# huyhoang17/DB_text_minimal

Hardware: AMD Instinct MI355X
Metric: train images/sec @640x640 bs=16/GPU (higher is better)
Workload: dtype f32

## Files before the change

db_text_minimal_amd/_lib.py:

```python
import ctypes
import os
import subprocess

_HERE = os.path.dirname(os.path.abspath(__file__))
LIB_PATH = os.environ.get('DBN_LIB_PATH') or os.path.join(_HERE, 'libdbnet_hip.so')
CSRC = os.path.join(_HERE, 'csrc')

_P, _I, _L, _F = ctypes.c_void_p, ctypes.c_int, ctypes.c_long, ctypes.c_float

SIGNATURES = {
    'dbn_pack_weights': 'piiiiiipp',
    'dbn_igemm_panel_floats': 'iiiiii',
    'dbn_igemm_packed_floats': 'ii',
    'dbn_igemm_f32': 'pppp' + 'i' * 14 + 'p',
    'dbn_igemm_tile_config': 'ii',
    'dbn_igemm_tile_config_ns': 'iii',
    'dbn_conv_bn_ws_floats': 'iiiiii',
    'dbn_pack_weights_batched': 'piip',
    'dbn_igemm_splitk_plan': 'iiii',
    'dbn_igemm_splitk_plan_ns': 'iiiii',
    'dbn_igemm_splitk_f32': 'pppp' + 'i' * 16 + 'pp',
    'dbn_deform_im2col': 'ppp' + 'i' * 11 + 'p',
    'dbn_deform_col2im': 'ppppp' + 'i' + 'p' + 'i' * 11 + 'p',
    'dbn_deform_col2im_ws_bytes': 'i' * 8,
# ... 180 lines not shown
    'dbn_convt16_rows': '',
    'dbn_convt16_panel_bytes': '',
    'dbn_convt16_eligible': 'iiiiii',
    'dbn_convt16_pack': 'ippp',
    'dbn_convt16_bn_t': 'ippppiii' + 'pp' + 'ff' + 'ppppppp' + 'p',
    'dbn_stem16_padded_h': 'i',
    'dbn_stem16_padded_w': 'i',
    'dbn_stem16_rows': '',
    'dbn_stem16_panel_bytes': '',
    'dbn_stem16_eligible': 'iiii',
    'dbn_stem16_pack': 'ippp',
    'dbn_nchw3_to_padded4_t': 'ipppiiip',
    'dbn_stem16_conv_bn_t': 'ipppiii' + 'pp' + 'ff' + 'ppppppp' + 'p',
    'dbn_head_tail_fwd_t': 'i' + SIGNATURES['dbn_head_tail_fwd'],
    'dbn_head_tail_bwd_t': 'i' + SIGNATURES['dbn_head_tail_bwd'],
})
LONG_RETURN = {'dbn_jpeg_coef_elems', 'dbn_jpeg_dhuff_ws_bytes', 'dbn_jpeg_encode_bound', 'dbn_greedy_decode_ws_bytes', 'dbn_det_eval_ws_bytes', 'dbn_detect_ws_bytes', 'dbn_detect_poly_ws_bytes', 'dbn_detect_poly_verts_cap', 'dbn_mfma_sustained_flops', 'dbn_conv_bn_final_group_doubles', 'dbn_maxpool_bn_backward_ws_floats', 'dbn_pw16_panel_bytes', 'dbn_stem16_panel_bytes', 'dbn_convt16_panel_bytes', 'dbn_winograd_panel_floats', 'dbn_winograd_wgrad_slab_floats', 'dbn_winograd_ws_floats', 'dbn_igemm_splitk_slab_floats', 'dbn_deform_col2im_ws_bytes', 'dbn_deform_col2im_gather_ws_bytes', 'dbn_igemm_bn_final_counters', 'dbn_igemm_bn_final_group_floats', 'dbn_igemm_panel_floats_t', 'dbn_wgrad_slab_floats_hw', 'dbn_wgrad_slab_floats', 'dbn_igemm_panel_floats', 'dbn_igemm_bf16s_panel_floats', 'dbn_db_loss_ohem_ws_bytes', 'dbn_conv_bn_ws_floats', 'dbn_pyramid_conv_ws_floats'}
_KIND = {'p': _P, 'i': _I, 'l': _L, 'f': _F}


class HipLibraryError(RuntimeError):
    pass


class WgradReduceJob(ctypes.Structure):
    _fields_ = ([('slab', _P), ('grad', _P)] + [(f, _I) for f in ('splitk', 'O', 'J', 'Jp', 'BM', 'BN', 'Cb', 'I', 'RS', 'G', 'natural', 'blocks')]
                + [('scale', _F), ('smem_bytes', _I)])


class BnbFinal(ctypes.Structure):
# ... 52 lines not shown
```

db_text_minimal_amd/csrc/common.h:

```cpp
#pragma once
#include <hip/hip_runtime.h>
#include <stdint.h>

typedef float f32x4 __attribute__((ext_vector_type(4)));
typedef float f32x16 __attribute__((ext_vector_type(16)));

#include <stdlib.h>

#ifdef DBN_EXPERIMENTS
#define DBN_HAS_EXPERIMENTS 1
static inline int dbn_env_int(const char* name, int dflt) { const char* e = getenv(name); return e ? atoi(e) : dflt; }
static inline double dbn_env_double(const char* name, double dflt) { const char* e = getenv(name); return e ? atof(e) : dflt; }
#else
#define DBN_HAS_EXPERIMENTS 0
static inline constexpr int dbn_env_int(const char*, int dflt) { return dflt; }
static inline constexpr double dbn_env_double(const char*, double dflt) { return dflt; }
#endif

#ifndef DBN_RACE
#define DBN_RACE 0
#endif
#if DBN_RACE
__device__ __forceinline__ void dbn_race_jitter(unsigned site) {
    unsigned h = (threadIdx.x >> 6) * 2654435761u + blockIdx.x * 40503u + site * 2246822519u;
// ... 60 lines not shown
    const float* row = part + idx * nb;
    double s = 0.0;
    int b = lane32;
    for (; b + 96 < nb; b += 128) {
        const float v0 = row[b], v1 = row[b + 32], v2 = row[b + 64], v3 = row[b + 96];
        s += ((double)v0 + (double)v1) + ((double)v2 + (double)v3);
    }
    for (; b < nb; b += 32) s += (double)row[b];
#pragma unroll
    for (int o = 16; o > 0; o >>= 1) s += __shfl_xor(s, o, 64);
    return s;
}

__device__ __forceinline__ float dbn_affine(float y, float sc, float sh) { return fmaf(y, sc, sh); }
__device__ __forceinline__ float dbn_affine_relu(float y, float sc, float sh) { return fmaxf(fmaf(y, sc, sh), 0.f); }

#define DBN_AT_F32 0
#define DBN_AT_BF16 1
#define DBN_AT_F16 2
typedef unsigned dbn_u32x2 __attribute__((ext_vector_type(2)));
typedef _Float16 dbn_f16x4 __attribute__((ext_vector_type(4)));
typedef __bf16 dbn_bf16x2 __attribute__((ext_vector_type(2)));

__host__ __device__ constexpr int dbn_esize(int at) { return at == 0 ? 4 : 2; }

template <int AT>
__device__ __forceinline__ f32x4 dbn_ld4(const void* __restrict__ p, long i4) {
    if constexpr (AT == 0) {
        return reinterpret_cast<const f32x4*>(p)[i4];
    } else if constexpr (AT == 1) {
// ... 86 lines not shown
```

db_text_minimal_amd/csrc/head_loss.hip:

```cpp
#include "common.h"

namespace {

__device__ __forceinline__ float sigmoidf_(float x) { return 1.f / (1.f + __expf(-x)); }
__device__ __forceinline__ float sigmoid_acc(float x) { return 1.f / (1.f + expf(-x)); }
__device__ __forceinline__ float sigmoid_fast(float x) { return __builtin_amdgcn_rcpf(1.f + __expf(-x)); }

template <int CTRL>
__device__ __forceinline__ float dpp_f32(float v) {
    return __builtin_bit_cast(float, __builtin_amdgcn_update_dpp(0, __builtin_bit_cast(int, v), CTRL, 0xF, 0xF, true));
}
constexpr int DPP_QUAD_XOR1 = 0xB1;
constexpr int DPP_QUAD_XOR2 = 0x4E;
constexpr int DPP_ROW_HALF_MIRROR = 0x141;
constexpr int DPP_ROW_MIRROR = 0x140;
__device__ __forceinline__ float group16_sum(float v) {
    v += dpp_f32<DPP_QUAD_XOR1>(v);
    v += dpp_f32<DPP_QUAD_XOR2>(v);
    v += dpp_f32<DPP_ROW_HALF_MIRROR>(v);
    v += dpp_f32<DPP_ROW_MIRROR>(v);
    return v;
}
#ifndef DBN_HT_NODPP
#define DBN_HT_NODPP 0
// ... 122 lines not shown
        }
    }
    for (; px < r1; px += gstride, advance()) {
        f32x4 vb[NQ], vt[NQ];
        load(xb, px, vb);
        load(xt, px, vt);
        finish(vb, vt, n, hq, wq);
    }
}

#if DBN_HT_WAVES
#define DBN_HT_OCC __attribute__((amdgpu_waves_per_eu(DBN_HT_WAVES, DBN_HT_WAVES)))
#else
#define DBN_HT_OCC
#endif
template <int AT>
__global__ __launch_bounds__(256) DBN_HT_OCC void head_tail_bwd_kernel(const void* __restrict__ xb, const void* __restrict__ xt, const float* __restrict__ wb,
                                     const float* __restrict__ wt, const float* __restrict__ preds,
                                     const float* __restrict__ dpreds, const float* __restrict__ sc_b,
                                     const float* __restrict__ sh_b, const float* __restrict__ sc_t,
                                     const float* __restrict__ sh_t, const float* __restrict__ mean_b,
                                     const float* __restrict__ rstd_b, const float* __restrict__ mean_t,
                                     const float* __restrict__ rstd_t, void* __restrict__ dxb, void* __restrict__ dxt,
                                     float* __restrict__ part, int N, int Hq, int Wq, int CH, float kstep) {
    const int q = threadIdx.x & 15;
    const int grp = threadIdx.x >> 4;
    const bool bn = sc_b != nullptr;
    f32x4 scb = {1.f, 1.f, 1.f, 1.f}, shb = {0.f, 0.f, 0.f, 0.f}, sct = scb, sht = shb;
    if (bn) {
        scb = *reinterpret_cast<const f32x4*>(sc_b + 4 * q);
        shb = *reinterpret_cast<const f32x4*>(sh_b + 4 * q);
        sct = *reinterpret_cast<const f32x4*>(sc_t + 4 * q);
        sht = *reinterpret_cast<const f32x4*>(sh_t + 4 * q);
    }
    const long npx = (long)N * Hq * Wq;
    const long gstride = (long)gridDim.x * (blockDim.x >> 4);
    f32x4 wbq[4], wtq[4];
#pragma unroll
    for (int e = 0; e < 4; ++e) {
// ... 52 lines not shown
        const f32x4 lb = {quad_bcast<0>(dlb), quad_bcast<1>(dlb), quad_bcast<2>(dlb), quad_bcast<3>(dlb)};
        const f32x4 lt = {quad_bcast<0>(dlt), quad_bcast<1>(dlt), quad_bcast<2>(dlt), quad_bcast<3>(dlt)};
        f32x4 vb = dbn_ld4<AT>(xb, px * 16 + q);
        f32x4 vt = dbn_ld4<AT>(xt, px * 16 + q);
        const f32x4 yb = vb, yt = vt;
        if (bn) {
#pragma unroll
            for (int e = 0; e < 4; ++e) {
                vb[e] = dbn_affine_relu(vb[e], scb[e], shb[e]);
                vt[e] = dbn_affine_relu(vt[e], sct[e], sht[e]);
            }
        }
        f32x4 gb, gt;
#pragma unroll
        for (int e = 0; e < 4; ++e) {
            gb[e] = wbq[e][0] * lb[0] + wbq[e][1] * lb[1] + wbq[e][2] * lb[2] + wbq[e][3] * lb[3];
            gt[e] = wtq[e][0] * lt[0] + wtq[e][1] * lt[1] + wtq[e][2] * lt[2] + wtq[e][3] * lt[3];
            awb[e] += vb[e] * lb;
            awt[e] += vt[e] * lt;
        }
        dbn_st4<AT>(dxb, px * 16 + q, gb);
        dbn_st4<AT>(dxt, px * 16 + q, gt);
        if (bnsum) {
            if constexpr (AT != 0) {
#pragma unroll
                for (int e = 0; e < 4; ++e) {
                    gb[e] = AT == 1 ? (float)(__bf16)gb[e] : (float)(_Float16)gb[e];
                    gt[e] = AT == 1 ? (float)(__bf16)gt[e] : (float)(_Float16)gt[e];
                }
            }
#pragma unroll
            for (int e = 0; e < 4; ++e) {
                const float mb = vb[e] > 0.f ? gb[e] : 0.f, mt = vt[e] > 0.f ? gt[e] : 0.f;
                s1b[e] += mb;
                s2b[e] += mb * ((yb[e] - mub[e]) * rsb[e]);
                s1t[e] += mt;
                s2t[e] += mt * ((yt[e] - mut[e]) * rst[e]);
// ... 540 lines not shown
        hipLaunchKernelGGL((head_tail_fwd_kernel<0, 16>), grid, dim3(256), 0, (hipStream_t)stream, xb, xt, wb, wt, bias_b, bias_t, bn_scale_b,
                           bn_shift_b, bn_scale_t, bn_shift_t, out, N, Hq, Wq, channels, kstep, per);
    else
        return DBN_ERR_ARG;
    return dbn_status();
}
int dbn_head_tail_fwd(const float* xb, const float* xt, const float* wb, const float* wt, const float* bias_b,
                      const float* bias_t, const float* bn_scale_b, const float* bn_shift_b, const float* bn_scale_t,
                      const float* bn_shift_t, float* out, int N, int Hq, int Wq, int channels, float kstep, void* stream) {
    return dbn_head_tail_fwd_t(0, xb, xt, wb, wt, bias_b, bias_t, bn_scale_b, bn_shift_b, bn_scale_t, bn_shift_t, out, N, Hq, Wq,
                               channels, kstep, stream);
}

int dbn_head_tail_bwd_ws_floats() { return 2048 * (2 * 257 + 4 * 64); }

int dbn_head_tail_bwd_t(int at, const void* xb, const void* xt, const float* wb, const float* wt, const float* preds,
                        const float* dpreds, const float* bn_scale_b, const float* bn_shift_b, const float* bn_scale_t,
                        const float* bn_shift_t, const float* bn_mean_b, const float* bn_rstd_b, const float* bn_mean_t,
                        const float* bn_rstd_t, float* bn_sums, void* dxb, void* dxt, float* dw_b, float* dbias_b, float* dw_t,
                        float* dbias_t, int N, int Hq, int Wq, int channels, float kstep, float grad_scale, float* ws, void* stream) {
    DBN_REQUIRE(xb && xt && wb && wt && preds && dpreds && dxb && dxt && dw_b && dbias_b && dw_t && dbias_t && ws);
    DBN_REQUIRE((bn_scale_b && bn_shift_b && bn_scale_t && bn_shift_t) || (!bn_scale_b && !bn_shift_b && !bn_scale_t && !bn_shift_t));
    DBN_REQUIRE(channels == 2 || channels == 3);
    const bool sums = bn_sums != nullptr;
    DBN_REQUIRE(!sums || (bn_scale_b && bn_mean_b && bn_rstd_b && bn_mean_t && bn_rstd_t));
    hipStream_t st = (hipStream_t)stream;
    const long npx = (long)N * Hq * Wq;
    const int nb = dbn_grid(npx * 16, 256, 2047);
    DBN_DISPATCH_AT(at, hipLaunchKernelGGL(head_tail_bwd_kernel<AT>, dim3(nb), dim3(256), 0, st, xb, xt, wb, wt, preds, dpreds, bn_scale_b,
                                           bn_shift_b, bn_scale_t, bn_shift_t, sums ? bn_mean_b : nullptr, bn_rstd_b, bn_mean_t,
                                           bn_rstd_t, dxb, dxt, ws, N, Hq, Wq, channels, kstep));
    hipLaunchKernelGGL(fold_head_grads_kernel, dim3(dbn_ceil_div(2 * 257, 8)), dim3(256), 0, st, ws, nb, dw_b, dbias_b, dw_t, dbias_t,
                       grad_scale);
    if (sums)
        hipLaunchKernelGGL(fold_partials_d_kernel, dim3(dbn_ceil_div(256, 8)), dim3(256), 0, st, ws + (long)514 * nb, nb, 256, bn_sums,
                           1.0f);
    return dbn_status();
}

int dbn_head_tail_bwd(const float* xb, const float* xt, const float* wb, const float* wt, const float* preds,
                      const float* dpreds, const float* bn_scale_b, const float* bn_shift_b, const float* bn_scale_t,
                      const float* bn_shift_t, const float* bn_mean_b, const float* bn_rstd_b, const float* bn_mean_t,
                      const float* bn_rstd_t, float* bn_sums, float* dxb, float* dxt, float* dw_b, float* dbias_b, float* dw_t,
                      float* dbias_t, int N, int Hq, int Wq, int channels, float kstep, float grad_scale, float* ws, void* stream) {
    return dbn_head_tail_bwd_t(0, xb, xt, wb, wt, preds, dpreds, bn_scale_b, bn_shift_b, bn_scale_t, bn_shift_t, bn_mean_b, bn_rstd_b,
                               bn_mean_t, bn_rstd_t, bn_sums, dxb, dxt, dw_b, dbias_b, dw_t, dbias_t, N, Hq, Wq, channels, kstep,
                               grad_scale, ws, stream);
}

static const long DB_LOSS_PART_BYTES = 1024L * NSUM * 8;
int dbn_db_loss_ws_bytes() { return (int)DB_LOSS_PART_BYTES + 64; }

// ... 96 lines not shown
```

db_text_minimal_amd/csrc/pointwise.hip:

```cpp
#include "common.h"

namespace {

constexpr int MAX_PART = 1024;
constexpr int STREAM_BLOCKS = 768;
constexpr int UNROLL = 4;

constexpr int CHUNK_C = 1024;

template <int NV, class F>
__device__ __forceinline__ void channel_reduce(int M, int Cfull, float* __restrict__ part, F&& body) {
    const int cb = blockIdx.y * CHUNK_C, C = min(CHUNK_C, Cfull - cb);
    const int c4n = C >> 2, cq = cb >> 2;
    const int c4 = threadIdx.x % c4n, rl = threadIdx.x / c4n;
    const int nrl = blockDim.x / c4n;
    const int rows_per = (M + gridDim.x - 1) / gridDim.x;
    const int r0 = blockIdx.x * rows_per, r1 = min(M, r0 + rows_per);
    f32x4 acc[NV];
#pragma unroll
    for (int v = 0; v < NV; ++v) acc[v] = f32x4{0.f, 0.f, 0.f, 0.f};
    if (rl < nrl) {
#pragma unroll 4
        for (int r = r0 + rl; r < r1; r += nrl) body(r, cq + c4, acc);
    }
// ... 217 lines not shown
    s1 = red[0][0];
    s2 = red[1][0];
    dbeta[c] = (float)(s1 * gscale);
    dgamma[c] = (float)(s2 * gscale);
    c1[c] = (float)(s1 / M);
    c2[c] = (float)(s2 / M);
}

template <int AT>
__device__ __forceinline__ float round_to_storage(float v) {
    if constexpr (AT == 1) return (float)(__bf16)v;
    else if constexpr (AT == 2) return (float)(_Float16)v;
    else return v;
}

template <int AT, int QW>
__global__ __launch_bounds__(256) void bn_bwd_apply_kernel(const void* __restrict__ y, const void* __restrict__ zmask,
                                                           const float* __restrict__ msc, const float* __restrict__ msh,
                                                           const void* __restrict__ dout, const float* __restrict__ mean,
                                                           const float* __restrict__ rstd, const float* __restrict__ gamma,
                                                           const float* __restrict__ c1, const float* __restrict__ c2,
                                                           void* __restrict__ dy, void* __restrict__ gout, int gout_acc,
                                                           long total, int C, float* __restrict__ bias_part) {
    static_assert(QW == 1 || (QW == 2 && AT != 0), "two quads per access: 16-bit storage");
    const int cin = C / (4 * QW);
    const long i0 = blockIdx.x * (long)blockDim.x + threadIdx.x;
    const long stride = (long)gridDim.x * blockDim.x;
    const int c = (int)(i0 % cin) * 4 * QW;
    const f32x4 zero = {0.f, 0.f, 0.f, 0.f};
    f32x4 s_[QW], h_[QW], mu[QW], rs[QW], k1[QW], k2[QW], gr[QW], bsum[QW];
#pragma unroll
    for (int q = 0; q < QW; ++q) {
        s_[q] = h_[q] = zero;
        if (msc) {
            s_[q] = *reinterpret_cast<const f32x4*>(msc + c + 4 * q);
            h_[q] = *reinterpret_cast<const f32x4*>(msh + c + 4 * q);
        }
        mu[q] = *reinterpret_cast<const f32x4*>(mean + c + 4 * q);
        rs[q] = *reinterpret_cast<const f32x4*>(rstd + c + 4 * q);
        k1[q] = *reinterpret_cast<const f32x4*>(c1 + c + 4 * q);
        k2[q] = *reinterpret_cast<const f32x4*>(c2 + c + 4 * q);
        gr[q] = *reinterpret_cast<const f32x4*>(gamma + c + 4 * q) * rs[q];
        bsum[q] = zero;
    }
    const bool acc = gout && gout_acc;
    auto ld = [&](const void* ptr, long i, f32x4 (&v)[QW]) {
        if constexpr (QW == 1) v[0] = dbn_ld4<AT>(ptr, i);
        else dbn_ldq<AT>(ptr, i, v);
    };
    auto st = [&](void* ptr, long i, const f32x4 (&v)[QW]) {
        if constexpr (QW == 1) dbn_st4<AT>(ptr, i, v[0]);
        else dbn_stq<AT>(ptr, i, v);
    };
    auto one = [&](long i, f32x4 (&g)[QW], const f32x4 (&v)[QW], const f32x4 (&z)[QW], const f32x4 (&old)[QW]) {
        f32x4 d[QW], go[QW];
#pragma unroll
        for (int q = 0; q < QW; ++q) {
            if (zmask) {
#pragma unroll
                for (int e = 0; e < 4; ++e) g[q][e] = z[q][e] > 0.f ? g[q][e] : 0.f;
            } else if (msc) {
#pragma unroll
                for (int e = 0; e < 4; ++e) g[q][e] = dbn_affine(v[q][e], s_[q][e], h_[q][e]) > 0.f ? g[q][e] : 0.f;
            }
            const f32x4 xh = (v[q] - mu[q]) * rs[q];
            d[q] = gr[q] * (g[q] - k1[q] - xh * k2[q]);
#pragma unroll
            for (int e = 0; e < 4; ++e) {
                float t = d[q][e];
                asm("" : "+v"(t));
// ... 2 lines not shown
            bsum[q] += d[q];
            go[q] = acc ? g[q] + old[q] : g[q];
        }
        st(dy, i, d);
        if (gout) st(gout, i, go);
    };
    auto zeros = [&](f32x4 (&v)[QW]) {
#pragma unroll
        for (int q = 0; q < QW; ++q) v[q] = zero;
    };
    long i = i0;
    for (; i + (UNROLL - 1) * stride < total; i += UNROLL * stride) {
        f32x4 g[UNROLL][QW], v[UNROLL][QW], z[UNROLL][QW], o[UNROLL][QW];
#pragma unroll
        for (int u = 0; u < UNROLL; ++u) {
            ld(dout, i + u * stride, g[u]);
            ld(y, i + u * stride, v[u]);
        }
#pragma unroll
        for (int u = 0; u < UNROLL; ++u) {
            if (zmask) ld(zmask, i + u * stride, z[u]);
            else zeros(z[u]);
            if (acc) ld(gout, i + u * stride, o[u]);
            else zeros(o[u]);
        }
#pragma unroll
        for (int u = 0; u < UNROLL; ++u) one(i + u * stride, g[u], v[u], z[u], o[u]);
    }
    for (; i < total; i += stride) {
        f32x4 g[QW], v[QW], z[QW], o[QW];
        ld(dout, i, g);
        ld(y, i, v);
        if (zmask) ld(zmask, i, z);
        else zeros(z);
        if (acc) ld(gout, i, o);
        else zeros(o);
        one(i, g, v, z, o);
    }
    if (bias_part) {
        __shared__ f32x4 red[QW][256];
#pragma unroll
        for (int q = 0; q < QW; ++q) red[q][threadIdx.x] = bsum[q];
        __syncthreads();
        if ((int)threadIdx.x < cin) {
            const int cq = (int)((blockIdx.x * (long)blockDim.x + threadIdx.x) % cin) * 4 * QW;
#pragma unroll
// ... 785 lines not shown
        } else if (sums) {
            hipLaunchKernelGGL(bn_bwd_finalize_kernel, dim3(dbn_ceil_div(C, 8)), dim3(256), 0, st, sums, sums_parts > 0 ? sums_parts : 1, M,
                               C, dgamma, dbeta, c1, c2, grad_scale);
        } else {
            hipLaunchKernelGGL(bn_bwd_reduce_kernel<AT>, red_grid(nbu, C), dim3(256), red_smem(C, 2), st, y, zmask, mask_scale,
                               mask_shift, dout, save_mean, save_rstd, M, C, ws);
            hipLaunchKernelGGL(bn_bwd_finalize_kernel, dim3(dbn_ceil_div(C, 8)), dim3(256), 0, st, ws, nbu, M, C, dgamma, dbeta, c1, c2,
                               grad_scale);
        }
#ifndef DBN_DBG_SKIP_BN_BWD_APPLY
#define DBN_DBG_SKIP_BN_BWD_APPLY 0
#endif
        if constexpr (AT != 0) {
            if (wide && !DBN_DBG_SKIP_BN_BWD_APPLY)
                hipLaunchKernelGGL((bn_bwd_apply_kernel<AT, 2>), dim3(grid), dim3(256), 0, st, y, zmask, mask_scale, mask_shift, dout, save_mean,
                                   save_rstd, gamma, c1, c2, dy, gout, gout_accumulate, total4, C, dbias_conv ? ws : nullptr);
        }
        if (!wide && !DBN_DBG_SKIP_BN_BWD_APPLY)
            hipLaunchKernelGGL((bn_bwd_apply_kernel<AT, 1>), dim3(grid), dim3(256), 0, st, y, zmask, mask_scale, mask_shift, dout, save_mean,
                               save_rstd, gamma, c1, c2, dy, gout, gout_accumulate, total4, C, dbias_conv ? ws : nullptr);
    });
    if (dbias_conv)
        hipLaunchKernelGGL(fold_partials_kernel, dim3(dbn_ceil_div(C, 8)), dim3(256), 0, st, ws, grid, C, dbias_conv, grad_scale);
    return dbn_status();
}

int dbn_bn_backward(const float* y, const float* zmask, const float* mask_scale, const float* mask_shift, const float* dout,
                    const float* save_mean, const float* save_rstd, const float* gamma, float* dy, float* gout, int gout_accumulate,
                    float* dgamma, float* dbeta, int M, int C, float grad_scale, float* ws, void* stream) {
    return dbn_bn_backward_t(0, nullptr, 0, y, zmask, mask_scale, mask_shift, dout, save_mean, save_rstd, gamma, dy, gout, gout_accumulate,
                             dgamma, dbeta, nullptr, M, C, grad_scale, ws, stream);
}

int dbn_bn_backward_from_sums(const float* sums, const float* y, const float* zmask, const float* mask_scale, const float* mask_shift,
                              const float* dout, const float* save_mean, const float* save_rstd, const float* gamma, float* dy,
                              float* gout, int gout_accumulate, float* dgamma, float* dbeta, int M, int C, float grad_scale,
// ... 264 lines not shown
```

db_text_minimal_amd/engine.py:

```python
import contextlib
import os

import torch

from . import _lib
from ._lib import check

DEAD_PREFIXES = ('backbone.fc.', 'backbone.smooth.')
K_STEP_DEFAULT = 50.0


def _p(t):
    return None if t is None else t.data_ptr()


def flat_layout(numels):
    offs, total = [], 0
    for n in numels:
        offs.append(total)
        total += (n + 3) // 4 * 4
    return offs, total


IGEMM_TILE_NAMES = {1: 'igemm_f32_kernel<128,128,2,2,%d,%d,%d,%s,%d,%s>', 2: 'igemm_f32_kernel<256,64,4,1,%d,%d,%d,%s,%d,%s>',
# ... 1051 lines not shown
            at, srcp = self._src(x.data_ptr(), C)
            check(self.L.dbn_igemm_act_t(at, self.ns, srcp, wpk.data_ptr(), vconv.bias.data_ptr(), _p(res), int(relu), z.data_ptr(), N, H, W, C,
                                         Ho, Wo, conv.cout, k, k, s, p, 0, 0, self.stream), 'igemm act ' + name)
        if self.prof:
            self.prof.end()
        return z

    apply_on_load = os.environ.get('DBN_APPLY_ON_LOAD', '1') == '1'
    fpn_level0_winograd = os.environ.get('DBN_FPN_LV0_WINOGRAD', '1') == '1'

    def lazy_act(self, y, convs, train):
        return all(self.plan(conv, y.shape, train, fp32_tensors=y.dtype == torch.float32).apply_on_load for conv in convs)

    bias_grad_in_bn = True

    def bn_backward(self, name, y, mask, dout, dy_name, gout=None, gout_acc=False, sums=None, conv_bias=None, sums_parts=1):
        self._flush_wgrads()
        C = y.shape[-1]
        M = y.numel() // C
        dy = self.buf(dy_name, *y.shape)
        zmask = msc = msh = None
        if isinstance(mask, str):
            msc, msh = self.bufs[name + '/scale'], self.bufs[name + '/shift']
        elif mask is not None:
            zmask = mask
        if sums is None and name in self._bnb_sums:
            sums, sums_parts = self._bnb_sums.pop(name)
        dbias = None
        if conv_bias is not None and self.bias_grad_in_bn and 256 % (C // 4) == 0:
            dbias = self.grad_views[conv_bias]
            self._bias_done.add(conv_bias)
        nb = y.numel() * y.element_size()
        rd = 2 + (zmask is not None)
        self._prof_hbm('bn_bwd_reduce_kernel + bn_bwd_finalize_kernel + bn_bwd_apply_kernel', nb * ((0 if sums is not None else rd) + rd + 1 + (gout is not None) * (1 + bool(gout_acc))),
                       name + (' [sums given]' if sums is not None else ''))
        check(self.L.dbn_bn_backward_t(self.at, _p(sums), int(sums_parts), y.data_ptr(), _p(zmask), _p(msc), _p(msh), dout.data_ptr(),
                                        self.bufs[name + '/mean'].data_ptr(), self.bufs[name + '/rstd'].data_ptr(),
                                        self.views[name + '.weight'].data_ptr(), dy.data_ptr(), _p(gout), int(gout_acc),
                                        self.grad_views[name + '.weight'].data_ptr(), self.grad_views[name + '.bias'].data_ptr(),
                                        _p(dbias), M, C, self.grad_scale, self.reduce_ws().data_ptr(), self.stream),
              'bn backward ' + name)
        if self.prof:
            self.prof.end()
        return dy

    def up_fwd(self, src, addend, dst, coff=0):
        N, Hs, Ws, C = src.shape
        _, H, W, Cd = dst.shape
# ... 454 lines not shown
            check(self.L.dbn_winograd_conv_act_f32(zs[0].data_ptr(), up.data_ptr(), vconv.bias.data_ptr(), None, 0, z.data_ptr(), N, H, W, Cg, Co,
                                                   self.stream), 'winograd ' + name)
            if self.prof:
                self.prof.end()
        if self.prof:
            flops = sum(2.0 * N * t.shape[1] * t.shape[2] * Cg * Co * ((1 << g) + 2)**2 for g, t in enumerate(zs) if g >= first)
            bn_tile = 256 if self.L.dbn_pyramid_wide_would_run(self.at, N, H, W, Cg, Co) else 128
            waves = '1,4' if (self.at in (1, 2) and self.ns == 1) else '2,2'
            self.prof.begin('igemm_f32_kernel<128,%d,%s,3,%d,%d,false,0,true>' % (bn_tile, waves, self.ns, self.at), flops, 0.0, 'fwd %s (pyramid)' % name)
        check(self.L.dbn_pyramid_conv_act_t(first, self.at, *[t.data_ptr() for t in zs], *[w_.data_ptr() for w_ in wpk], vconv.bias.data_ptr(), 1,
                                            z.data_ptr(), N, H, W, Cg, Co, self.ns, self.stream), 'pyramid_conv_act')
        if self.prof:
            self.prof.end()
        return z

    def backward(self, dpreds):
        if self.saved_generation != self.generation:
            raise RuntimeError('backward() without a matching train-mode forward (activations were overwritten)')
        m, L, st = self.model, self.L, self.stream
        N, H, W, Hh, Wh, resample = self.saved_shape
        B = self.bufs
        self._bias_done = set()
        self._bnb_sums = {}
        self._dcn_read_back()
        self._wgrad_fifo, self._reduce_pending = [], []
        self._slab_free = [None, None]
        out = self.saved_out
        dpreds = dpreds.contiguous()
        assert dpreds.shape == (N, 3, H, W)
        if resample:
            dhead = self.fbuf('head/dout', *out.shape)
            check(L.dbn_bilinear_bwd(dpreds.data_ptr(), dhead.data_ptr(), N * 3, 2 * Hh, 2 * Wh, H, W, st), 'bilinear_bwd')
            dpreds = dhead
        head = m.segmentation_head
        b6, t6 = head.binarize[6], head.thresh[6]
        dz1b = self.buf('binarize/dz1', N, Hh, Wh, 64)
        dz1t = self.buf('thresh/dz1', N, Hh, Wh, 64)
        ws = self.scratch('_head_ws', L.dbn_head_tail_bwd_ws_floats())
        G = self.grad_views
        hb, ht = 'segmentation_head.binarize.4', 'segmentation_head.thresh.4'
        bn_sums = self.fbuf('head/bn4_sums', 4, 64)
        self._prof_hbm('head_tail_bwd_kernel + fold_head_grads_kernel + fold_partials_d_kernel', 4.0 * dz1b.element_size() * dz1b.numel() + 4.0 * (out.numel() + dpreds.numel()))
        check(L.dbn_head_tail_bwd_t(self.at, B['binarize/y1'].data_ptr(), B['thresh/y1'].data_ptr(), b6.weight.data_ptr(),
                                  t6.weight.data_ptr(), out.data_ptr(), dpreds.data_ptr(), B[hb + '/scale'].data_ptr(),
                                  B[hb + '/shift'].data_ptr(), B[ht + '/scale'].data_ptr(), B[ht + '/shift'].data_ptr(),
                                  B[hb + '/mean'].data_ptr(), B[hb + '/rstd'].data_ptr(), B[ht + '/mean'].data_ptr(),
                                  B[ht + '/rstd'].data_ptr(), bn_sums.data_ptr(), dz1b.data_ptr(), dz1t.data_ptr(),
                                  G['segmentation_head.binarize.6.weight'].data_ptr(),
                                  G['segmentation_head.binarize.6.bias'].data_ptr(),
                                  G['segmentation_head.thresh.6.weight'].data_ptr(),
                                  G['segmentation_head.thresh.6.bias'].data_ptr(), N, Hh, Wh, 3, float(head.k),
                                  self.grad_scale, ws.data_ptr(), st), 'head_tail_bwd')
        if self.prof:
            self.prof.end()
        f, f_act = B.get('fpn/z'), None
        if f is None:
            f, f_act = B['fpn/y'], (B['segmentation_body.conv.1/scale'], B['segmentation_body.conv.1/shift'])
        df = self.buf('fpn/dz', *f.shape)
        fpn = m.segmentation_body
        pre = 'segmentation_body.'
        for i, (br, dz1) in enumerate((('binarize', dz1b), ('thresh', dz1t))):
            seq = getattr(head, br)
            hp = 'segmentation_head.%s.' % br
            dy1 = self.bn_backward(hp + '4', B[br + '/y1'], 'self', dz1, br + '/dy1', sums=bn_sums[2 * i:2 * i + 2],
                                   conv_bias=hp + '3.bias' if seq[3].bias is not None else None)
            dz0 = self.buf(br + '/dz0', *B[br + '/z0'].shape)
            self.convT_bwd(hp + '3', dy1, B[br + '/z0'], seq[3], dz0, consumer=(hp + '1', B[br + '/y0'], None))
            dy0 = self.bn_backward(hp + '1', B[br + '/y0'], 'self', dz0, br + '/dy0',
                                   conv_bias=hp + '0.bias' if seq[0].bias is not None else None)
            self.conv_wgrad(hp + '0', dy0, f, seq[0], x_act=f_act)
            self.conv_dgrad(hp + '0', dy0, seq[0], df, accumulate=(i > 0),
                            consumer=(pre + 'conv.1', B['fpn/y'], None) if i > 0 else None)
        fpn = m.segmentation_body
        pre = 'segmentation_body.'
        dfy = self.bn_backward(pre + 'conv.1', B['fpn/y'], 'self', df, 'fpn/dy',
                               conv_bias=pre + 'conv.0.bias' if fpn.conv[0].bias is not None else None)
        dP = {}
        levels = ('smooth_p2', 'smooth_p3', 'smooth_p4', 'reduce_conv_c5')
        zs = [B[nm + '/z'] for nm in levels]
        if self.fpn_exact:
# ... 277 lines not shown
```

include/dbnet_hip.h:

```cpp
#ifndef DBNET_HIP_H
#define DBNET_HIP_H
#ifdef __cplusplus
extern "C" {
#endif


int dbn_pack_weights(const float* w_oihw, int O, int I, int R, int S, int mode, int stride, float* out, void* stream);
long dbn_igemm_panel_floats(int O, int I, int R, int S, int mode, int stride);
int dbn_igemm_packed_floats(int K, int Cd);

int dbn_igemm_f32(const float* src, const float* wpk, const float* bias, float* dst, int N, int Hs, int Ws, int Cs, int Hd,
                  int Wd, int Cd, int R, int S, int stride, int pad, int mode, int accumulate, int tile_hint, void* stream);

int dbn_pack_weights_bf16s(const float* w_oihw, int O, int I, int R, int S, int mode, int stride, int ns, float* out, void* stream);
int dbn_pack_weights_batched(const void* jobs, int n, int ns, void* stream);
long dbn_igemm_bf16s_panel_floats(int O, int I, int R, int S, int mode, int stride, int ns);
int dbn_igemm_bf16s(const float* src, const float* wpk, const float* bias, float* dst, int N, int Hs, int Ws, int Cs, int Hd,
                    int Wd, int Cd, int R, int S, int stride, int pad, int mode, int accumulate, int tile_hint, int ns,
                    void* stream);
int dbn_wgrad_bf16s(const float* sm, const float* big, float* slab, float* grad_oihw, int N, int Ho, int Wo, int O, int H, int W,
                    int Cb, int I, int R, int S, int stride, int pad, float scale, int ns, void* stream);

int dbn_igemm_bn_rows(int at, int ns, int N, int Hs, int Ws, int Cs, int Hd, int Wd, int Cd, int R, int S, int stride, int pad, int mode,
                      int tile_hint);
// ... 349 lines not shown
                           const float* bias1_t, const float* scale_b, const float* shift_b, const float* scale_t, const float* shift_t,
                           const float* w2_b, const float* w2_t, const float* bias2_b, const float* bias2_t, float* out, int N, int Hq, int Wq,
                           void* stream);

int dbn_nchw3_to_nhwc16_and_4_t(int at, const float* x, void* out16, void* out4, int N, int H, int W, void* stream);
int dbn_nchw3_to_nhwc4_packed_t(int at, const float* x, void* out, int N, int H, int W, void* stream);
int dbn_head_tail_fwd_t(int at, const void* xb, const void* xt, const float* wb, const float* wt, const float* bias_b,
                        const float* bias_t, const float* bn_scale_b, const float* bn_shift_b, const float* bn_scale_t,
                        const float* bn_shift_t, float* out, int N, int Hq, int Wq, int channels, float kstep, void* stream);
int dbn_set_head_tail_wide(int mode);
int dbn_head_tail_bwd_t(int at, const void* xb, const void* xt, const float* wb, const float* wt, const float* preds,
                        const float* dpreds, const float* bn_scale_b, const float* bn_shift_b, const float* bn_scale_t,
                        const float* bn_shift_t, const float* bn_mean_b, const float* bn_rstd_b, const float* bn_mean_t,
                        const float* bn_rstd_t, float* bn_sums, void* dxb, void* dxt, float* dw_b, float* dbias_b, float* dw_t,
                        float* dbias_t, int N, int Hq, int Wq, int channels, float kstep, float grad_scale, float* ws, void* stream);

int dbn_jpeg_info(const unsigned char* data, long len, long long* out);
long dbn_jpeg_coef_elems(const unsigned char* blob, const long long* offs, int N, long long* per_image);
int dbn_jpeg_entropy_batch(const unsigned char* blob, const long long* offs, int N, short* coef, long coef_elems, long long* desc,
                           unsigned short* qtabs, int* status, int threads);
int dbn_jpeg_pixels(const short* coef, long coef_elems, const long long* desc, const unsigned short* qtabs, int N, const int* tab_idct,
                    int n_idct, const int* tab_rgb, int n_rgb, unsigned char* planes, unsigned char* out, long out_bytes, void* stream);

int dbn_jpeg_forward(const unsigned char* pixels, long in_bytes, const long long* desc, const unsigned short* qtabs, int N,
                     const int* tab_planes, int n_planes, const int* tab_fdct, int n_fdct, unsigned char* planes, short* coef, long coef_elems,
                     void* stream);
long dbn_jpeg_encode_bound(const long long* desc, int N, int restart_interval, long long* per_image);
int dbn_jpeg_encode_batch(const short* coef, long coef_elems, const long long* desc, const unsigned short* qtabs, int N, int restart_interval,
                          unsigned char* out, long out_bytes, const long long* offs, long long* lens, int* status, int threads);
int dbn_jpeg_optimal_table(const long long* freq, unsigned char* bits, unsigned char* vals, int* nvals);
// ... 28 lines not shown
```

Baseline: 733.1.

## Pass 4-channel logit gradients to head BN backward and recompute 64-channel gradient

The head tail backward kernel can now write only the per-pixel 4-wide logit gradient instead of the full 64-channel input gradient. A new BN-backward variant rebuilds the 64-channel gradient on the fly from those logits and the final conv weights. This removes a large fp32 write and re-read of the dz1 tensors at half resolution, at the cost of a few extra FMAs per element in the BN apply kernel. The path is on by default for fp32 storage only.

New measurement: 740.3 (median of 6 runs). About the same (+1.0%).

```diff
diff --git a/db_text_minimal_amd/_lib.py b/db_text_minimal_amd/_lib.py
--- a/db_text_minimal_amd/_lib.py
+++ b/db_text_minimal_amd/_lib.py
@@ -218,6 +218,8 @@
     'dbn_stem16_conv_bn_t': 'ipppiii' + 'pp' + 'ff' + 'ppppppp' + 'p',
     'dbn_head_tail_fwd_t': 'i' + SIGNATURES['dbn_head_tail_fwd'],
     'dbn_head_tail_bwd_t': 'i' + SIGNATURES['dbn_head_tail_bwd'],
+    'dbn_head_tail_bwd_dl_t': 'i' + SIGNATURES['dbn_head_tail_bwd'],
+    'dbn_bn_backward_headgrad_t': 'ipi' + 'p' * 11 + 'i' + 'ppp' + 'ii' + 'f' + 'pp',
 })
 LONG_RETURN = {'dbn_jpeg_coef_elems', 'dbn_jpeg_dhuff_ws_bytes', 'dbn_jpeg_encode_bound', 'dbn_greedy_decode_ws_bytes', 'dbn_det_eval_ws_bytes', 'dbn_detect_ws_bytes', 'dbn_detect_poly_ws_bytes', 'dbn_detect_poly_verts_cap', 'dbn_mfma_sustained_flops', 'dbn_conv_bn_final_group_doubles', 'dbn_maxpool_bn_backward_ws_floats', 'dbn_pw16_panel_bytes', 'dbn_stem16_panel_bytes', 'dbn_convt16_panel_bytes', 'dbn_winograd_panel_floats', 'dbn_winograd_wgrad_slab_floats', 'dbn_winograd_ws_floats', 'dbn_igemm_splitk_slab_floats', 'dbn_deform_col2im_ws_bytes', 'dbn_deform_col2im_gather_ws_bytes', 'dbn_igemm_bn_final_counters', 'dbn_igemm_bn_final_group_floats', 'dbn_igemm_panel_floats_t', 'dbn_wgrad_slab_floats_hw', 'dbn_wgrad_slab_floats', 'dbn_igemm_panel_floats', 'dbn_igemm_bf16s_panel_floats', 'dbn_db_loss_ohem_ws_bytes', 'dbn_conv_bn_ws_floats', 'dbn_pyramid_conv_ws_floats'}
 _KIND = {'p': _P, 'i': _I, 'l': _L, 'f': _F}
diff --git a/db_text_minimal_amd/csrc/common.h b/db_text_minimal_amd/csrc/common.h
--- a/db_text_minimal_amd/csrc/common.h
+++ b/db_text_minimal_amd/csrc/common.h
@@ -98,6 +98,7 @@
 
 __device__ __forceinline__ float dbn_affine(float y, float sc, float sh) { return fmaf(y, sc, sh); }
 __device__ __forceinline__ float dbn_affine_relu(float y, float sc, float sh) { return fmaxf(fmaf(y, sc, sh), 0.f); }
+__device__ __forceinline__ float dbn_head_chan_grad(f32x4 w, f32x4 l) { return w[0] * l[0] + w[1] * l[1] + w[2] * l[2] + w[3] * l[3]; }
 
 #define DBN_AT_F32 0
 #define DBN_AT_BF16 1
diff --git a/db_text_minimal_amd/csrc/head_loss.hip b/db_text_minimal_amd/csrc/head_loss.hip
--- a/db_text_minimal_amd/csrc/head_loss.hip
+++ b/db_text_minimal_amd/csrc/head_loss.hip
@@ -160,7 +160,7 @@
 #else
 #define DBN_HT_OCC
 #endif
-template <int AT>
+template <int AT, bool DL>
 __global__ __launch_bounds__(256) DBN_HT_OCC void head_tail_bwd_kernel(const void* __restrict__ xb, const void* __restrict__ xt, const float* __restrict__ wb,
                                      const float* __restrict__ wt, const float* __restrict__ preds,
                                      const float* __restrict__ dpreds, const float* __restrict__ sc_b,
@@ -169,6 +169,7 @@
                                      const float* __restrict__ rstd_b, const float* __restrict__ mean_t,
                                      const float* __restrict__ rstd_t, void* __restrict__ dxb, void* __restrict__ dxt,
                                      float* __restrict__ part, int N, int Hq, int Wq, int CH, float kstep) {
+    static_assert(!DL || AT == 0, "logit-gradient output: fp32 storage");
     const int q = threadIdx.x & 15;
     const int grp = threadIdx.x >> 4;
     const bool bn = sc_b != nullptr;
@@ -251,13 +252,20 @@
         f32x4 gb, gt;
 #pragma unroll
         for (int e = 0; e < 4; ++e) {
-            gb[e] = wbq[e][0] * lb[0] + wbq[e][1] * lb[1] + wbq[e][2] * lb[2] + wbq[e][3] * lb[3];
-            gt[e] = wtq[e][0] * lt[0] + wtq[e][1] * lt[1] + wtq[e][2] * lt[2] + wtq[e][3] * lt[3];
+            gb[e] = dbn_head_chan_grad(wbq[e], lb);
+            gt[e] = dbn_head_chan_grad(wtq[e], lt);
             awb[e] += vb[e] * lb;
             awt[e] += vt[e] * lt;
         }
-        dbn_st4<AT>(dxb, px * 16 + q, gb);
-        dbn_st4<AT>(dxt, px * 16 + q, gt);
+        if constexpr (DL) {
+            if (q == 0) {
+                reinterpret_cast<f32x4*>(dxb)[px] = lb;
+                reinterpret_cast<f32x4*>(dxt)[px] = lt;
+            }
+        } else {
+            dbn_st4<AT>(dxb, px * 16 + q, gb);
+            dbn_st4<AT>(dxt, px * 16 + q, gt);
+        }
         if (bnsum) {
             if constexpr (AT != 0) {
 #pragma unroll
@@ -828,7 +836,7 @@
 
 int dbn_head_tail_bwd_ws_floats() { return 2048 * (2 * 257 + 4 * 64); }
 
-int dbn_head_tail_bwd_t(int at, const void* xb, const void* xt, const float* wb, const float* wt, const float* preds,
+static int head_tail_bwd_run(bool dl, int at, const void* xb, const void* xt, const float* wb, const float* wt, const float* preds,
                         const float* dpreds, const float* bn_scale_b, const float* bn_shift_b, const float* bn_scale_t,
                         const float* bn_shift_t, const float* bn_mean_b, const float* bn_rstd_b, const float* bn_mean_t,
                         const float* bn_rstd_t, float* bn_sums, void* dxb, void* dxt, float* dw_b, float* dbias_b, float* dw_t,
@@ -836,20 +844,46 @@
     DBN_REQUIRE(xb && xt && wb && wt && preds && dpreds && dxb && dxt && dw_b && dbias_b && dw_t && dbias_t && ws);
     DBN_REQUIRE((bn_scale_b && bn_shift_b && bn_scale_t && bn_shift_t) || (!bn_scale_b && !bn_shift_b && !bn_scale_t && !bn_shift_t));
     DBN_REQUIRE(channels == 2 || channels == 3);
+    DBN_REQUIRE(!dl || at == 0);
     const bool sums = bn_sums != nullptr;
     DBN_REQUIRE(!sums || (bn_scale_b && bn_mean_b && bn_rstd_b && bn_mean_t && bn_rstd_t));
     hipStream_t st = (hipStream_t)stream;
     const long npx = (long)N * Hq * Wq;
     const int nb = dbn_grid(npx * 16, 256, 2047);
-    DBN_DISPATCH_AT(at, hipLaunchKernelGGL(head_tail_bwd_kernel<AT>, dim3(nb), dim3(256), 0, st, xb, xt, wb, wt, preds, dpreds, bn_scale_b,
-                                           bn_shift_b, bn_scale_t, bn_shift_t, sums ? bn_mean_b : nullptr, bn_rstd_b, bn_mean_t,
-                                           bn_rstd_t, dxb, dxt, ws, N, Hq, Wq, channels, kstep));
+    if (dl)
+        hipLaunchKernelGGL((head_tail_bwd_kernel<0, true>), dim3(nb), dim3(256), 0, st, xb, xt, wb, wt, preds, dpreds, bn_scale_b, bn_shift_b,
+                           bn_scale_t, bn_shift_t, sums ? bn_mean_b : nullptr, bn_rstd_b, bn_mean_t, bn_rstd_t, dxb, dxt, ws, N, Hq, Wq, channels,
+                           kstep);
+    else
+        DBN_DISPATCH_AT(at, hipLaunchKernelGGL((head_tail_bwd_kernel<AT, false>), dim3(nb), dim3(256), 0, st, xb, xt, wb, wt, preds, dpreds,
+                                               bn_scale_b, bn_shift_b, bn_scale_t, bn_shift_t, sums ? bn_mean_b : nullptr, bn_rstd_b,
+                                               bn_mean_t, bn_rstd_t, dxb, dxt, ws, N, Hq, Wq, channels, kstep));
     hipLaunchKernelGGL(fold_head_grads_kernel, dim3(dbn_ceil_div(2 * 257, 8)), dim3(256), 0, st, ws, nb, dw_b, dbias_b, dw_t, dbias_t,
                        grad_scale);
     if (sums)
         hipLaunchKernelGGL(fold_partials_d_kernel, dim3(dbn_ceil_div(256, 8)), dim3(256), 0, st, ws + (long)514 * nb, nb, 256, bn_sums,
                            1.0f);
     return dbn_status();
+}
+
+int dbn_head_tail_bwd_t(int at, const void* xb, const void* xt, const float* wb, const float* wt, const float* preds,
+                        const float* dpreds, const float* bn_scale_b, const float* bn_shift_b, const float* bn_scale_t,
+                        const float* bn_shift_t, const float* bn_mean_b, const float* bn_rstd_b, const float* bn_mean_t,
+                        const float* bn_rstd_t, float* bn_sums, void* dxb, void* dxt, float* dw_b, float* dbias_b, float* dw_t,
+                        float* dbias_t, int N, int Hq, int Wq, int channels, float kstep, float grad_scale, float* ws, void* stream) {
+    return head_tail_bwd_run(false, at, xb, xt, wb, wt, preds, dpreds, bn_scale_b, bn_shift_b, bn_scale_t, bn_shift_t, bn_mean_b, bn_rstd_b,
+                             bn_mean_t, bn_rstd_t, bn_sums, dxb, dxt, dw_b, dbias_b, dw_t, dbias_t, N, Hq, Wq, channels, kstep, grad_scale,
+                             ws, stream);
+}
+
+int dbn_head_tail_bwd_dl_t(int at, const void* xb, const void* xt, const float* wb, const float* wt, const float* preds,
+                           const float* dpreds, const float* bn_scale_b, const float* bn_shift_b, const float* bn_scale_t,
+                           const float* bn_shift_t, const float* bn_mean_b, const float* bn_rstd_b, const float* bn_mean_t,
+                           const float* bn_rstd_t, float* bn_sums, float* dl_b, float* dl_t, float* dw_b, float* dbias_b, float* dw_t,
+                           float* dbias_t, int N, int Hq, int Wq, int channels, float kstep, float grad_scale, float* ws, void* stream) {
+    return head_tail_bwd_run(true, at, xb, xt, wb, wt, preds, dpreds, bn_scale_b, bn_shift_b, bn_scale_t, bn_shift_t, bn_mean_b, bn_rstd_b,
+                             bn_mean_t, bn_rstd_t, bn_sums, dl_b, dl_t, dw_b, dbias_b, dw_t, dbias_t, N, Hq, Wq, channels, kstep, grad_scale,
+                             ws, stream);
 }
 
 int dbn_head_tail_bwd(const float* xb, const float* xt, const float* wb, const float* wt, const float* preds,
diff --git a/db_text_minimal_amd/csrc/pointwise.hip b/db_text_minimal_amd/csrc/pointwise.hip
--- a/db_text_minimal_amd/csrc/pointwise.hip
+++ b/db_text_minimal_amd/csrc/pointwise.hip
@@ -255,14 +255,22 @@
     else return v;
 }
 
-template <int AT, int QW>
+template <bool HG>
+struct bn_head_grad_src {};
+template <>
+struct bn_head_grad_src<true> {
+    const float* dl;
+    const float* w6;
+};
+template <int AT, int QW, bool HG = false>
 __global__ __launch_bounds__(256) void bn_bwd_apply_kernel(const void* __restrict__ y, const void* __restrict__ zmask,
                                                            const float* __restrict__ msc, const float* __restrict__ msh,
                                                            const void* __restrict__ dout, const float* __restrict__ mean,
                                                            const float* __restrict__ rstd, const float* __restrict__ gamma,
                                                            const float* __restrict__ c1, const float* __restrict__ c2,
                                                            void* __restrict__ dy, void* __restrict__ gout, int gout_acc,
-                                                           long total, int C, float* __restrict__ bias_part) {
+                                                           long total, int C, float* __restrict__ bias_part, bn_head_grad_src<HG> hg) {
+    static_assert(!HG || (AT == 0 && QW == 1), "head gradient from the logit gradients: fp32 storage");
     static_assert(QW == 1 || (QW == 2 && AT != 0), "two quads per access: 16-bit storage");
     const int cin = C / (4 * QW);
     const long i0 = blockIdx.x * (long)blockDim.x + threadIdx.x;
@@ -285,9 +293,18 @@
         bsum[q] = zero;
     }
     const bool acc = gout && gout_acc;
+    f32x4 w6q[4];
+    if constexpr (HG) {
+#pragma unroll
+        for (int e = 0; e < 4; ++e) w6q[e] = *reinterpret_cast<const f32x4*>(hg.w6 + (c + e) * 4);
+    }
     auto ld = [&](const void* ptr, long i, f32x4 (&v)[QW]) {
         if constexpr (QW == 1) v[0] = dbn_ld4<AT>(ptr, i);
         else dbn_ldq<AT>(ptr, i, v);
+    };
+    auto ldg = [&](long i, f32x4 (&v)[QW]) {
+        if constexpr (HG) v[0] = reinterpret_cast<const f32x4*>(hg.dl)[i >> 4];
+        else ld(dout, i, v);
     };
     auto st = [&](void* ptr, long i, const f32x4 (&v)[QW]) {
         if constexpr (QW == 1) dbn_st4<AT>(ptr, i, v[0]);
@@ -295,6 +312,11 @@
     };
     auto one = [&](long i, f32x4 (&g)[QW], const f32x4 (&v)[QW], const f32x4 (&z)[QW], const f32x4 (&old)[QW]) {
         f32x4 d[QW], go[QW];
+        if constexpr (HG) {
+            const f32x4 l = g[0];
+#pragma unroll
+            for (int e = 0; e < 4; ++e) g[0][e] = dbn_head_chan_grad(w6q[e], l);
+        }
 #pragma unroll
         for (int q = 0; q < QW; ++q) {
             if (zmask) {
@@ -327,7 +349,7 @@
         f32x4 g[UNROLL][QW], v[UNROLL][QW], z[UNROLL][QW], o[UNROLL][QW];
 #pragma unroll
         for (int u = 0; u < UNROLL; ++u) {
-            ld(dout, i + u * stride, g[u]);
+            ldg(i + u * stride, g[u]);
             ld(y, i + u * stride, v[u]);
         }
 #pragma unroll
@@ -342,7 +364,7 @@
     }
     for (; i < total; i += stride) {
         f32x4 g[QW], v[QW], z[QW], o[QW];
-        ld(dout, i, g);
+        ldg(i, g);
         ld(y, i, v);
         if (zmask) ld(zmask, i, z);
         else zeros(z);
@@ -1158,12 +1180,36 @@
         if constexpr (AT != 0) {
             if (wide && !DBN_DBG_SKIP_BN_BWD_APPLY)
                 hipLaunchKernelGGL((bn_bwd_apply_kernel<AT, 2>), dim3(grid), dim3(256), 0, st, y, zmask, mask_scale, mask_shift, dout, save_mean,
-                                   save_rstd, gamma, c1, c2, dy, gout, gout_accumulate, total4, C, dbias_conv ? ws : nullptr);
+                                   save_rstd, gamma, c1, c2, dy, gout, gout_accumulate, total4, C, dbias_conv ? ws : nullptr, bn_head_grad_src<false>{});
         }
         if (!wide && !DBN_DBG_SKIP_BN_BWD_APPLY)
             hipLaunchKernelGGL((bn_bwd_apply_kernel<AT, 1>), dim3(grid), dim3(256), 0, st, y, zmask, mask_scale, mask_shift, dout, save_mean,
-                               save_rstd, gamma, c1, c2, dy, gout, gout_accumulate, total4, C, dbias_conv ? ws : nullptr);
+                               save_rstd, gamma, c1, c2, dy, gout, gout_accumulate, total4, C, dbias_conv ? ws : nullptr, bn_head_grad_src<false>{});
     });
+    if (dbias_conv)
+        hipLaunchKernelGGL(fold_partials_kernel, dim3(dbn_ceil_div(C, 8)), dim3(256), 0, st, ws, grid, C, dbias_conv, grad_scale);
+    return dbn_status();
+}
+
+int dbn_bn_backward_headgrad_t(int at, const float* sums, int sums_parts, const void* y, const void* zmask, const float* mask_scale,
+                               const float* mask_shift, const float* dl, const float* w6, const float* save_mean, const float* save_rstd,
+                               const float* gamma, void* dy, void* gout, int gout_accumulate, float* dgamma, float* dbeta,
+                               float* dbias_conv, int M, int C, float grad_scale, float* ws, void* stream) {
+    DBN_REQUIRE(at == 0 && C == 64 && M > 0);
+    DBN_REQUIRE(sums && sums_parts >= 0 && y && dl && w6 && save_mean && save_rstd && gamma && dy && dgamma && dbeta && ws);
+    DBN_REQUIRE(!zmask && !gout && !gout_accumulate && mask_scale && mask_shift);
+    hipStream_t st = (hipStream_t)stream;
+    float* c1 = ws + (long)MAX_PART * 2 * C - 2 * C;
+    float* c2 = c1 + C;
+    const long total4 = (long)M * (C / 4);
+    const int grid = bn_stream_grid(total4, C);
+    if (sums_parts >= 512)
+        hipLaunchKernelGGL(bn_bwd_finalize_wide_kernel, dim3(C), dim3(256), 0, st, sums, sums_parts, M, C, dgamma, dbeta, c1, c2, grad_scale);
+    else
+        hipLaunchKernelGGL(bn_bwd_finalize_kernel, dim3(dbn_ceil_div(C, 8)), dim3(256), 0, st, sums, sums_parts > 0 ? sums_parts : 1, M, C,
+                           dgamma, dbeta, c1, c2, grad_scale);
+    hipLaunchKernelGGL((bn_bwd_apply_kernel<0, 1, true>), dim3(grid), dim3(256), 0, st, y, nullptr, mask_scale, mask_shift, nullptr, save_mean,
+                       save_rstd, gamma, c1, c2, dy, nullptr, 0, total4, C, dbias_conv ? ws : nullptr, bn_head_grad_src<true>{dl, w6});
     if (dbias_conv)
         hipLaunchKernelGGL(fold_partials_kernel, dim3(dbn_ceil_div(C, 8)), dim3(256), 0, st, ws, grid, C, dbias_conv, grad_scale);
     return dbn_status();
diff --git a/db_text_minimal_amd/engine.py b/db_text_minimal_amd/engine.py
--- a/db_text_minimal_amd/engine.py
+++ b/db_text_minimal_amd/engine.py
@@ -1089,7 +1089,7 @@
 
     bias_grad_in_bn = True
 
-    def bn_backward(self, name, y, mask, dout, dy_name, gout=None, gout_acc=False, sums=None, conv_bias=None, sums_parts=1):
+    def bn_backward(self, name, y, mask, dout, dy_name, gout=None, gout_acc=False, sums=None, conv_bias=None, sums_parts=1, head_w6=None):
         self._flush_wgrads()
         C = y.shape[-1]
         M = y.numel() // C
@@ -1107,6 +1107,18 @@
             self._bias_done.add(conv_bias)
         nb = y.numel() * y.element_size()
         rd = 2 + (zmask is not None)
+        if head_w6 is not None:
+            assert mask == 'self' and gout is None and sums is not None, name
+            self._prof_hbm('bn_bwd_reduce_kernel + bn_bwd_finalize_kernel + bn_bwd_apply_kernel', 2 * nb + 4 * dout.numel(), name + ' [sums given]')
+            check(self.L.dbn_bn_backward_headgrad_t(self.at, sums.data_ptr(), int(sums_parts), y.data_ptr(), None, msc.data_ptr(), msh.data_ptr(),
+                                                    dout.data_ptr(), head_w6.data_ptr(), self.bufs[name + '/mean'].data_ptr(),
+                                                    self.bufs[name + '/rstd'].data_ptr(), self.views[name + '.weight'].data_ptr(),
+                                                    dy.data_ptr(), None, 0, self.grad_views[name + '.weight'].data_ptr(),
+                                                    self.grad_views[name + '.bias'].data_ptr(), _p(dbias), M, C, self.grad_scale,
+                                                    self.reduce_ws().data_ptr(), self.stream), 'bn backward (head gradient) ' + name)
+            if self.prof:
+                self.prof.end()
+            return dy
         self._prof_hbm('bn_bwd_reduce_kernel + bn_bwd_finalize_kernel + bn_bwd_apply_kernel', nb * ((0 if sums is not None else rd) + rd + 1 + (gout is not None) * (1 + bool(gout_acc))),
                        name + (' [sums given]' if sums is not None else ''))
         check(self.L.dbn_bn_backward_t(self.at, _p(sums), int(sums_parts), y.data_ptr(), _p(zmask), _p(msc), _p(msh), dout.data_ptr(),
@@ -1591,6 +1603,8 @@
             self.prof.end()
         return z
 
+    head_recompute = os.environ.get('DBN_HEAD_RECOMPUTE', '1') == '1'
+
     def backward(self, dpreds):
         if self.saved_generation != self.generation:
             raise RuntimeError('backward() without a matching train-mode forward (activations were overwritten)')
@@ -1611,14 +1625,21 @@
             dpreds = dhead
         head = m.segmentation_head
         b6, t6 = head.binarize[6], head.thresh[6]
-        dz1b = self.buf('binarize/dz1', N, Hh, Wh, 64)
-        dz1t = self.buf('thresh/dz1', N, Hh, Wh, 64)
+        recompute = self.head_recompute and self.at == 0
+        if recompute:
+            dz1b = self.fbuf('binarize/dl1', N, Hh, Wh, 4)
+            dz1t = self.fbuf('thresh/dl1', N, Hh, Wh, 4)
+        else:
+            dz1b = self.buf('binarize/dz1', N, Hh, Wh, 64)
+            dz1t = self.buf('thresh/dz1', N, Hh, Wh, 64)
         ws = self.scratch('_head_ws', L.dbn_head_tail_bwd_ws_floats())
         G = self.grad_views
         hb, ht = 'segmentation_head.binarize.4', 'segmentation_head.thresh.4'
         bn_sums = self.fbuf('head/bn4_sums', 4, 64)
-        self._prof_hbm('head_tail_bwd_kernel + fold_head_grads_kernel + fold_partials_d_kernel', 4.0 * dz1b.element_size() * dz1b.numel() + 4.0 * (out.numel() + dpreds.numel()))
-        check(L.dbn_head_tail_bwd_t(self.at, B['binarize/y1'].data_ptr(), B['thresh/y1'].data_ptr(), b6.weight.data_ptr(),
+        y1b = B['binarize/y1']
+        self._prof_hbm('head_tail_bwd_kernel + fold_head_grads_kernel + fold_partials_d_kernel',
+                       2.0 * y1b.element_size() * y1b.numel() + 2.0 * dz1b.element_size() * dz1b.numel() + 4.0 * (out.numel() + dpreds.numel()))
+        check((L.dbn_head_tail_bwd_dl_t if recompute else L.dbn_head_tail_bwd_t)(self.at, B['binarize/y1'].data_ptr(), B['thresh/y1'].data_ptr(), b6.weight.data_ptr(),
                                   t6.weight.data_ptr(), out.data_ptr(), dpreds.data_ptr(), B[hb + '/scale'].data_ptr(),
                                   B[hb + '/shift'].data_ptr(), B[ht + '/scale'].data_ptr(), B[ht + '/shift'].data_ptr(),
                                   B[hb + '/mean'].data_ptr(), B[hb + '/rstd'].data_ptr(), B[ht + '/mean'].data_ptr(),
@@ -1640,7 +1661,8 @@
             seq = getattr(head, br)
             hp = 'segmentation_head.%s.' % br
             dy1 = self.bn_backward(hp + '4', B[br + '/y1'], 'self', dz1, br + '/dy1', sums=bn_sums[2 * i:2 * i + 2],
-                                   conv_bias=hp + '3.bias' if seq[3].bias is not None else None)
+                                   conv_bias=hp + '3.bias' if seq[3].bias is not None else None,
+                                   head_w6=seq[6].weight if recompute else None)
             dz0 = self.buf(br + '/dz0', *B[br + '/z0'].shape)
             self.convT_bwd(hp + '3', dy1, B[br + '/z0'], seq[3], dz0, consumer=(hp + '1', B[br + '/y0'], None))
             dy0 = self.bn_backward(hp + '1', B[br + '/y0'], 'self', dz0, br + '/dy0',
diff --git a/include/dbnet_hip.h b/include/dbnet_hip.h
--- a/include/dbnet_hip.h
+++ b/include/dbnet_hip.h
@@ -387,6 +387,15 @@
                         const float* bn_shift_t, const float* bn_mean_b, const float* bn_rstd_b, const float* bn_mean_t,
                         const float* bn_rstd_t, float* bn_sums, void* dxb, void* dxt, float* dw_b, float* dbias_b, float* dw_t,
                         float* dbias_t, int N, int Hq, int Wq, int channels, float kstep, float grad_scale, float* ws, void* stream);
+int dbn_head_tail_bwd_dl_t(int at, const void* xb, const void* xt, const float* wb, const float* wt, const float* preds,
+                           const float* dpreds, const float* bn_scale_b, const float* bn_shift_b, const float* bn_scale_t,
+                           const float* bn_shift_t, const float* bn_mean_b, const float* bn_rstd_b, const float* bn_mean_t,
+                           const float* bn_rstd_t, float* bn_sums, float* dl_b, float* dl_t, float* dw_b, float* dbias_b, float* dw_t,
+                           float* dbias_t, int N, int Hq, int Wq, int channels, float kstep, float grad_scale, float* ws, void* stream);
+int dbn_bn_backward_headgrad_t(int at, const float* sums, int sums_parts, const void* y, const void* zmask, const float* mask_scale,
+                               const float* mask_shift, const float* dl, const float* w6, const float* save_mean, const float* save_rstd,
+                               const float* gamma, void* dy, void* gout, int gout_accumulate, float* dgamma, float* dbeta,
+                               float* dbias_conv, int M, int C, float grad_scale, float* ws, void* stream);
 
 int dbn_jpeg_info(const unsigned char* data, long len, long long* out);
 long dbn_jpeg_coef_elems(const unsigned char* blob, const long long* offs, int N, long long* per_image);
```
